# seung-lab/crackle

Hardware: AMD Instinct MI355X
Metric: voxels/s encode+decode, 1024x1024x512 uint32; bit-exact .ckl bytes (higher is better)
Workload: dtype u32

## Files before the change

crackle_amd/csrc/ckl_encode.hip:

```cpp
#include "ckl_common.hpp"
#include "ckl_runs.hpp"
#include "ckl_trail.hpp"
#include "ckl_pins_dev.hpp"

#include <algorithm>
#include <atomic>
#include <chrono>
#include <functional>
#include <memory>
#include <mutex>

namespace ckl {

using namespace dev;

template <typename LABEL>
__global__ void __launch_bounds__(kBlock) k_stats(const LABEL* __restrict__ labels, uint64_t voxels, unsigned long long* __restrict__ out ) {
	__shared__ unsigned long long s_max[kWaves], s_pairs[kWaves];
	unsigned long long mx = 0, pairs = 0;
	const uint64_t stride = static_cast<uint64_t>(gridDim.x) * kBlock;
	for (uint64_t i = static_cast<uint64_t>(blockIdx.x) * kBlock + threadIdx.x; i < voxels; i += stride) {
		const LABEL v = labels[i];
		if (static_cast<unsigned long long>(v) > mx) mx = v;
		if (i > 0) pairs += (labels[i - 1] == v);
// ... 631 lines not shown
	uint32_t b = planeV[wi];
	if (w == 0) b |= 1u;
	const uint32_t* cc = run_cc + rbase[zi];
	const uint32_t add = static_cast<uint32_t>(comp_off[zi]) + id_base;
	uint32_t run = word_base[wi] - 1u + __popc(b & (0xFFFFFFFFu >> (31u - bit)));
	uint4 o;
	o.x = cc[run] + add;
	run += (b >> (bit + 1u)) & 1u; o.y = cc[run] + add;
	run += (b >> (bit + 2u)) & 1u; o.z = cc[run] + add;
	run += (b >> (bit + 3u)) & 1u; o.w = cc[run] + add;
	*reinterpret_cast<uint4*>(out + zi * sxy + px) = o;
}

inline void launch_paint_components(hipStream_t s, const uint32_t* planeV, uint32_t row_words, uint64_t plane_words, int64_t sx, int64_t sy, int64_t sz,
	const uint32_t* word_base, const uint64_t* rbase, const uint32_t* run_cc, const uint64_t* comp_off, uint32_t id_base, uint32_t* out) {
	const uint64_t sxy = static_cast<uint64_t>(sx) * sy;
	const bool four = sx % 4 == 0 && (reinterpret_cast<uintptr_t>(out) & 15u) == 0;
	const uint64_t threads = four ? sxy / 4 : sxy;
	const dim3 grid(static_cast<uint32_t>((threads + kBlock - 1) / kBlock), static_cast<uint32_t>(sz));
	if (four) hipLaunchKernelGGL(k_paint_components4, grid, dim3(kBlock), 0, s, planeV, row_words, plane_words, static_cast<uint32_t>(sx), sxy, word_base, rbase, run_cc, comp_off, id_base, out);
	else hipLaunchKernelGGL(k_paint_components, grid, dim3(kBlock), 0, s, planeV, row_words, plane_words, static_cast<uint32_t>(sx), sxy, word_base, rbase, run_cc, comp_off, id_base, out);
}

__global__ void __launch_bounds__(kBlock) k_bitonic_step(uint64_t* __restrict__ a, uint32_t j, uint32_t k, uint32_t n) {
	const uint32_t i = blockIdx.x * kBlock + threadIdx.x;
	if (i >= n) return;
	const uint32_t l = i ^ j;
	if (l > i) {
		const uint64_t x = a[i], y = a[l];
		const bool up = (i & k) == 0;
		if ((x > y) == up) { a[i] = y; a[l] = x; }
	}
}
__global__ void __launch_bounds__(kBlock) k_bitonic_step2(uint64_t* __restrict__ a, uint32_t j, uint32_t k, uint32_t n) {
	const uint32_t t = blockIdx.x * kBlock + threadIdx.x;
	if (t >= n / 4u) return;
	const uint32_t h = j >> 1;
	const uint32_t lb = static_cast<uint32_t>(__ffs(h)) - 1u;
	const uint32_t i = (t & (h - 1u)) | ((t >> lb) << (lb + 2u));
	uint64_t v0 = a[i], v1 = a[i | h], v2 = a[i | j], v3 = a[i | j | h];
	const bool up = (i & k) == 0;
	auto cx = [&](uint64_t& x, uint64_t& y) { if ((x > y) == up) { const uint64_t z = x; x = y; y = z; } };
	cx(v0, v2); cx(v1, v3);
	cx(v0, v1); cx(v2, v3);
	a[i] = v0; a[i | h] = v1; a[i | j] = v2; a[i | j | h] = v3;
}

__global__ void __launch_bounds__(kBlock) k_bitonic_first(uint64_t* __restrict__ a, uint32_t n) {
	__shared__ uint64_t s[2048];
	const uint32_t base = blockIdx.x * 2048u;
	for (uint32_t t = threadIdx.x; t < 2048u; t += kBlock) s[t] = base + t < n ? a[base + t] : ~0ull;
	__syncthreads();
	for (uint32_t k = 2; k <= 2048u; k <<= 1) {
		for (uint32_t j = k >> 1; j > 0; j >>= 1) {
			for (uint32_t t = threadIdx.x; t < 2048u; t += kBlock) {
				const uint32_t l = t ^ j;
				if (l > t) {
					const uint64_t x = s[t], y = s[l];
					const bool up = ((base + t) & k) == 0;
					if ((x > y) == up) { s[t] = y; s[l] = x; }
				}
			}
			__syncthreads();
		}
	}
	for (uint32_t t = threadIdx.x; t < 2048u; t += kBlock) if (base + t < n) a[base + t] = s[t];
}
__global__ void __launch_bounds__(kBlock) k_bitonic_local(uint64_t* __restrict__ a, uint32_t j_start, uint32_t k, uint32_t n) {
	__shared__ uint64_t s[2048];
	const uint32_t base = blockIdx.x * 2048u;
	for (uint32_t t = threadIdx.x; t < 2048u; t += kBlock) s[t] = base + t < n ? a[base + t] : ~0ull;
	__syncthreads();
	for (uint32_t j = j_start; j > 0; j >>= 1) {
		for (uint32_t t = threadIdx.x; t < 2048u; t += kBlock) {
			const uint32_t l = t ^ j;
			if (l > t) {
				const uint64_t x = s[t], y = s[l];
				const bool up = ((base + t) & k) == 0;
				if ((x > y) == up) { s[t] = y; s[l] = x; }
			}
		}
		__syncthreads();
	}
	for (uint32_t t = threadIdx.x; t < 2048u; t += kBlock) if (base + t < n) a[base + t] = s[t];
}
__global__ void __launch_bounds__(kBlock) k_pad_copy_u64(const uint64_t* __restrict__ src, uint64_t n, uint64_t* __restrict__ dst, uint64_t n_pad) {
	const uint64_t i = static_cast<uint64_t>(blockIdx.x) * kBlock + threadIdx.x;
	if (i < n_pad) dst[i] = i < n ? src[i] : ~0ull;
}
constexpr uint32_t kUniqPer = 8, kUniqItems = kBlock * kUniqPer;
__device__ __forceinline__ uint32_t unique_heads(const uint64_t* __restrict__ sorted, uint32_t n, uint32_t i0, uint64_t (&v)[kUniqPer]) {
	uint32_t flag = 0;
#pragma unroll
	for (uint32_t q = 0; q < kUniqPer; q++) {
		const uint32_t i = i0 + q;
		v[q] = i < n ? sorted[i] : 0;
		const uint64_t prev = q ? v[q - 1] : ((i > 0 && i < n) ? sorted[i - 1] : 0);
		flag |= ((i < n && (i == 0 || v[q] != prev)) ? 1u : 0u) << q;
	}
	return flag;
}
__global__ void __launch_bounds__(kBlock) k_unique_count(const uint64_t* __restrict__ sorted, uint32_t n, uint32_t* __restrict__ blk_count) {
	__shared__ uint32_t s_red[kWaves];
	uint64_t v[kUniqPer];
	const uint32_t flag = unique_heads(sorted, n, blockIdx.x * kUniqItems + threadIdx.x * kUniqPer, v);
	const uint32_t tot = block_sum(static_cast<uint32_t>(__popc(flag)), s_red);
	if (threadIdx.x == 0) blk_count[blockIdx.x] = tot;
}
__global__ void __launch_bounds__(kBlock) k_unique_scan(uint32_t* __restrict__ blk_count, uint32_t nblk, uint32_t* __restrict__ n_uniq) {
	__shared__ uint32_t s_scan[kWaves];
	uint32_t carry = 0;
// ... 50 lines not shown
__global__ void __launch_bounds__(kBlock) k_label_hash_count(const unsigned long long* __restrict__ table, uint32_t slots, uint32_t* __restrict__ blk_count) {
	__shared__ uint32_t s_red[kWaves];
	uint64_t v[kUniqPer];
	const uint32_t flag = hash_occupied(table, slots, blockIdx.x * kUniqItems + threadIdx.x * kUniqPer, v);
	const uint32_t tot = block_sum(static_cast<uint32_t>(__popc(flag)), s_red);
	if (threadIdx.x == 0) blk_count[blockIdx.x] = tot;
}
__global__ void __launch_bounds__(kBlock) k_label_hash_scatter(
	const unsigned long long* __restrict__ table, uint32_t slots, const uint32_t* __restrict__ blk_base, const uint32_t* __restrict__ n_found,
	const uint32_t* __restrict__ has_max, uint64_t* __restrict__ out
) {
	__shared__ uint32_t s_scan[kWaves];
	uint64_t v[kUniqPer];
	const uint32_t flag = hash_occupied(table, slots, blockIdx.x * kUniqItems + threadIdx.x * kUniqPer, v);
	uint32_t c[1] = { static_cast<uint32_t>(__popc(flag)) }, tot[1];
	block_excl_add<1>(c, tot, s_scan);
	uint32_t o = blk_base[blockIdx.x] + c[0];
#pragma unroll
	for (uint32_t q = 0; q < kUniqPer; q++) if ((flag >> q) & 1u) out[o++] = v[q];
	if (blockIdx.x == 0 && threadIdx.x == 0 && *has_max) out[*n_found] = kLabelHashEmpty;
}

__global__ void __launch_bounds__(kBlock) k_flat_section(
	const uint64_t* __restrict__ uniq, const uint32_t* __restrict__ n_uniq, int stored_width,
	const uint32_t* __restrict__ ncomp, uint32_t nslices, int component_width,
	const uint64_t* __restrict__ mapping, uint32_t n, uint8_t* __restrict__ out
) {
	const uint32_t nu = *n_uniq;
	const int key_width = nu <= 0xFFu ? 1 : (nu <= 0xFFFFu ? 2 : 4);
	const uint32_t i = blockIdx.x * kBlock + threadIdx.x;
	if (i == 0) for (int b = 0; b < 8; b++) out[b] = static_cast<uint8_t>((static_cast<uint64_t>(nu) >> (8 * b)) & 0xFF);
	uint8_t* o_uniq = out + 8;
	uint8_t* o_cc = o_uniq + static_cast<uint64_t>(nu) * stored_width;
	uint8_t* o_keys = o_cc + static_cast<uint64_t>(nslices) * component_width;
	if (i < nu) {
		const uint64_t v = uniq[i];
		for (int b = 0; b < stored_width; b++) o_uniq[static_cast<uint64_t>(i) * stored_width + b] = static_cast<uint8_t>((v >> (8 * b)) & 0xFF);
	}
	if (i < nslices) {
		const uint32_t v = ncomp[i];
		for (int b = 0; b < component_width; b++) o_cc[static_cast<uint64_t>(i) * component_width + b] = b < 4 ? static_cast<uint8_t>((v >> (8 * b)) & 0xFF) : 0;
	}
	if (i < n) {
		const uint64_t v = mapping[i];
		uint32_t lo = 0, hi = nu;
		while (lo + 1 < hi) {
			const uint32_t mid = (lo + hi) >> 1;
			if (uniq[mid] <= v) lo = mid; else hi = mid;
		}
		for (int b = 0; b < key_width; b++) o_keys[static_cast<uint64_t>(i) * key_width + b] = static_cast<uint8_t>((lo >> (8 * b)) & 0xFF);
	}
// ... 170 lines not shown
	hipStream_t stream_tab = nullptr;
	hipEvent_t ev_codes = nullptr;
	void* tables_staging = nullptr;
	bool uploads_by_kernel = false;
	hipEvent_t ev_labels_crc = nullptr;
	DevBuf<uint32_t> d_labels_crc;
	DevBuf<uint8_t> d_stream_out;
	uint64_t device_stream_bytes = 0;
	uint64_t last_codes_total = 0;
	DevBuf<uint32_t> d_stack_node, d_stack_code;
	DevBuf<uint32_t> d_chain_node, d_chain_off, d_chain_clen, d_chain_order, d_chain_dst, d_chain_vstart;
	DevBuf<uint32_t> d_n_chains, d_n_raw, d_n_valid, d_payload_len, d_boc_len;
	DevBuf<uint32_t> d_hist;
	DevBuf<uint32_t> d_planes, d_count_vh;
	uint32_t row_words = 0;
	uint64_t plane_words = 0;
	std::vector<uint32_t> count_v, count_h;
	DevBuf<uint64_t> d_rbase;
	DevBuf<uint32_t> d_rcap, d_word_base, d_parent, d_run_start, d_run_cc, d_comp_pix, d_nruns, d_ncomp, d_idbits, d_blk_roots;
	DevBuf<uint16_t> d_run_local;
	DevBuf<uint32_t> d_G, d_crc_acc;
	DevBuf<uint32_t> d_flat_report;
	uint64_t g_table_pixels = 0;
	DevBuf<uint64_t> d_mapping, d_sorted, d_uniq, d_label_hash, d_label_list;
	DevBuf<uint8_t> d_keys;
	DevBuf<uint32_t> d_cc_volume;
	DevBuf<uint32_t> d_pin_kept, d_pin_u32;
	DevBuf<uint8_t> d_pin_tables;
	DevBuf<uint64_t> d_pin_u64;
	DevBuf<uint32_t> d_slice_err2, d_n_uniq, d_uniq_blk;
	DevBuf<uint8_t> d_labels_bin;
	uint32_t flat_max_rcap = 0;
	const void* planes_for = nullptr;
	const void* trail_for = nullptr;
	bool trail_perm = false;
	int trail_order = 0;
	VolumeStats planes_stats;
	int64_t planes_dims[3] = { 0, 0, 0 };
	std::vector<uint64_t> h_rbase;
	std::vector<uint32_t> h_rcap;
	std::vector<uint32_t> count_special, count_corner;
	DevBuf<uint32_t> d_plane_partial, t_blk_special, t_blk_corner;
	DevBuf<unsigned long long> d_plane_partial_max, d_plane_out;
	uint32_t graph_blocks = 0;
	uint32_t tiles_x = 0, tiles_y = 0, mtx2 = 0;
	uint64_t adjm_stride = 0;
	bool graph_permissible = false;
	bool planes_deferred = false;
	bool trail_zeroed = false;
	DevBuf<uint64_t> t_nbase, t_cobase, t_ibase;
	DevBuf<uint32_t> t_ncap, t_cocap, t_icap, t_max_steps;
	size_t last_trail_slices = 0;
	DevBuf<uint32_t> t_counters;
	DevBuf<uint32_t> t_node_vertex, t_vert2node, t_corner_vertex;
	DevBuf<uint8_t> t_node_adj;
	DevBuf<uint32_t> t_dart_end, t_dart_len, t_dart_minv, t_dart_minpos, t_parent, t_start_bits, t_starts;
	DevBuf<uint4> t_dart_codes;
	DevBuf<uint8_t> t_dart_inline;
	DevBuf<unsigned long long> t_compmin;
	DevBuf<uint32_t> t_items, t_item_off, t_chain_item0, t_events, t_chain_ev0, t_ev_lnd, t_ev_item;

	~ckl_encoder() {
		if (ev0) (void)hipEventDestroy(ev0);
		if (ev1) (void)hipEventDestroy(ev1);
		if (evk0) (void)hipEventDestroy(evk0);
		if (evk1) (void)hipEventDestroy(evk1);
		if (evd0) (void)hipEventDestroy(evd0);
		if (evd1) (void)hipEventDestroy(evd1);
		if (ev_in) (void)hipEventDestroy(ev_in);
		if (ev_prezero) (void)hipEventDestroy(ev_prezero);
		if (stream) (void)hipStreamDestroy(stream);
		if (stream2) (void)hipStreamDestroy(stream2);
		if (stream_copy) { (void)hipStreamSynchronize(stream_copy); (void)hipStreamDestroy(stream_copy); }
		if (stream_tab) { (void)hipStreamSynchronize(stream_tab); (void)hipStreamDestroy(stream_tab); }
		if (ev_codes) (void)hipEventDestroy(ev_codes);
		if (tables_staging) host_out_free(tables_staging);
		if (ev_labels_crc) (void)hipEventDestroy(ev_labels_crc);
	}
};

namespace {

template <typename T>
void upload(DevBuf<T>& d, const std::vector<T>& h, hipStream_t s) {
	d.ensure(h.size());
	if (!h.empty()) CKL_HIP(hipMemcpyAsync(d.p, h.data(), h.size() * sizeof(T), hipMemcpyHostToDevice, s));
}
struct UploadPacker {
	struct Item { void* buf; size_t off, count; void (*bind)(void*, uint8_t*, size_t); };
	std::vector<Item> items;
	std::vector<uint8_t> image;
	template <typename T>
	void add(DevBuf<T>& dst, const std::vector<T>& src) {
		const size_t off = (image.size() + 255) & ~static_cast<size_t>(255);
		image.resize(off + std::max<size_t>(src.size(), 1) * sizeof(T));
// ... 527 lines not shown
		const std::vector<uint32_t> rep = download(e.d_flat_report.p, 4 * static_cast<size_t>(ns), s);
		out.ncomp.assign(rep.begin(), rep.begin() + ns);
		acc.assign(rep.begin() + ns, rep.begin() + 2 * static_cast<size_t>(ns));
		idbits.assign(rep.begin() + 2 * static_cast<size_t>(ns), rep.begin() + 3 * static_cast<size_t>(ns));
		errs.assign(rep.begin() + 3 * static_cast<size_t>(ns), rep.end());
		HT_MARK("f:wait");
	}
	else {
		out.ncomp = download(e.d_ncomp.p, ns, s);
		HT_MARK("f:wait");
		acc = download(e.d_crc_acc.p, ns, s);
		idbits = download(e.d_idbits.p, ns, s);
		errs = download(e.d_slice_err2.p, ns, s);
	}
	for (uint32_t zi = 0; zi < ns; zi++) if (errs[zi]) throw Error(CKL_ERR_RUNTIME, "crackle_amd: run table overflow on z=" + std::to_string(zi));
	const uint32_t init_term = gf_mul(0xFFFFFFFFu, gf_xpow(32ull * sxy));
	out.crcs.resize(ns);
	uint32_t fix_bits = 0xFFFFFFFFu, fix = 0;
	for (uint32_t zi = 0; zi < ns; zi++) {
		if (idbits[zi] != fix_bits) { fix_bits = idbits[zi]; fix = gf_xpow(32 - fix_bits); }
		out.crcs[zi] = ~(gf_mul(acc[zi], fix) ^ init_term);
	}

	std::vector<uint64_t> comp_off(ns);
	uint64_t total = 0;
	for (uint32_t zi = 0; zi < ns; zi++) { comp_off[zi] = total; total += out.ncomp[zi]; }
	upload(e.d_comp_off, comp_off, s);
	e.d_mapping.ensure(total + 1);
	RunArrays ra;
	ra.word_base = e.d_word_base.p; ra.rbase = e.d_rbase.p; ra.rcap = e.d_rcap.p;
	ra.parent = e.d_parent.p; ra.run_start = e.d_run_start.p; ra.run_cc = e.d_run_cc.p;
	ra.nruns = e.d_nruns.p; ra.ncomp = e.d_ncomp.p; ra.slice_err = e.d_slice_err2.p;
	ra.comp_pix = e.d_comp_pix.p;
	uint32_t max_ncomp = 1;
	for (uint32_t zi = 0; zi < ns; zi++) max_ncomp = std::max(max_ncomp, out.ncomp[zi]);
	hipLaunchKernelGGL(k_mapping_comps<LABEL>, dim3((max_ncomp + kBlock - 1) / kBlock, ns), dim3(kBlock), 0, s,
		labels, ra, sxy, e.d_comp_off.p, e.d_mapping.p);
	CKL_HIP(hipStreamSynchronize(s));
	out.total = total;
}

struct PinLabelLists {
	DevBuf<uint64_t> d_tab;
	DevBuf<uint32_t> d_count;
	uint32_t slots = 0;
	hipEvent_t ready = nullptr;
	~PinLabelLists() { if (ready) (void)hipEventDestroy(ready); }
};
void pin_label_table_enqueue(ckl_encoder& e, const uint64_t* comp_label, const uint64_t* first_any_dev, uint64_t N, PinLabelLists& t) {
	hipStream_t s = e.stream2;
	if (N > (1ull << 30)) throw Error(CKL_ERR_RUNTIME, "crackle_amd: too many components for pin labels");
	uint32_t slots = 1024;
	while (slots < 2 * N) slots <<= 1;
	t.slots = slots;
	t.d_tab.ensure(4ull * slots + 1);
	t.d_count.ensure(1);
	CKL_HIP(hipMemsetAsync(t.d_tab.p, 0xFF, (2ull * slots) * sizeof(uint64_t), s));
	CKL_HIP(hipMemsetAsync(t.d_tab.p + 4ull * slots, 0xFF, sizeof(uint64_t), s));
	CKL_HIP(hipMemsetAsync(t.d_count.p, 0, sizeof(uint32_t), s));
	unsigned long long* tab = reinterpret_cast<unsigned long long*>(t.d_tab.p);
	hipLaunchKernelGGL(k_pin_label_first, dim3(static_cast<uint32_t>((N + kPinBlock - 1) / kPinBlock)), dim3(kPinBlock), 0, s,
// ... 346 lines not shown
		pin_label_table_collect(e, lists, lc);
		HT_MARK("p:lists");
		table = pins_label_table_host(lc.label_value, lc.label_first);
		HT_MARK("p:table");
	}
	const uint64_t total = download(d_off.p + N, 1, s)[0];
	HT_MARK("p:passes");
	uint64_t id_budget = 1ull << 26;
	if (const char* env = getenv("CKL_PIN_IDS_BUDGET")) id_budget = static_cast<uint64_t>(std::max(0, atoi(env)));
	if (total > id_budget || getenv("CKL_PINS_HOST_BOOKKEEPING")) {
		const PinCandidates pc = pin_candidates_device<LABEL>(e, labels, cc, comp_label, sx, sy, sz, N, &v, choice, first_any);
		HT_MARK("pins_device");
		return pins_cover_host(pc, sx, sy, sz, nc, N, index_width, stored_width, auto_bgcolor, manual_bgcolor);
	}
	d_ze.ensure(N); d_ids.ensure(total + 1);
	hipLaunchKernelGGL(k_pin_minus1, dim3(nb), dim3(kPinBlock), 0, s, d_zep.p, N, d_ze.p);
	hipLaunchKernelGGL(k_pin_ids, dim3(nb), dim3(kPinBlock), 0, s, v, choice, d_ze.p, reinterpret_cast<const uint64_t*>(d_off.p), static_cast<uint32_t>(N), d_ids.p);
	std::vector<uint8_t> bin = pins_section_from_device(e, sx, sy, sz, N, nc, comp_label, first_any, reinterpret_cast<const uint64_t*>(choice), d_zep.p,
		reinterpret_cast<const uint64_t*>(d_off.p), d_ids.p, stored_width, auto_bgcolor, manual_bgcolor, table.get());
	HT_MARK("pins_host");
	return bin;
}

uint64_t flat_section(ckl_encoder& e, uint64_t N, int stored_width, int component_width, uint32_t ns, const ckl_encode_overrides* ov = nullptr) {
	hipStream_t s = e.stream2;
	if (N > 0x7FFFFFFFull) throw Error(CKL_ERR_RUNTIME, "crackle_amd: too many components");
	e.d_n_uniq.ensure(2);
	e.d_uniq.ensure(N + 1);
	const uint64_t* sort_src = e.d_mapping.p;
	uint64_t n_sort = N;
	if (N > 8192 && N <= (1ull << 26) && !getenv("CKL_LABEL_SORT_ALL")) {
		uint32_t slots = 16384;
		while (slots < 2 * N) slots <<= 1;
		e.d_label_hash.ensure(slots);
		CKL_HIP(hipMemsetAsync(e.d_label_hash.p, 0xFF, static_cast<size_t>(slots) * sizeof(uint64_t), s));
		CKL_HIP(hipMemsetAsync(e.d_n_uniq.p, 0, 2 * sizeof(uint32_t), s));
		unsigned long long* table = reinterpret_cast<unsigned long long*>(e.d_label_hash.p);
		hipLaunchKernelGGL(k_label_hash_insert, dim3(static_cast<uint32_t>((N + kBlock - 1) / kBlock)), dim3(kBlock), 0, s, e.d_mapping.p, static_cast<uint32_t>(N), table, slots - 1u, e.d_n_uniq.p + 1);
		const uint32_t hb = (slots + kUniqItems - 1) / kUniqItems;
		e.d_uniq_blk.ensure(hb + 1);
		hipLaunchKernelGGL(k_label_hash_count, dim3(hb), dim3(kBlock), 0, s, table, slots, e.d_uniq_blk.p);
		hipLaunchKernelGGL(k_unique_scan, dim3(1), dim3(kBlock), 0, s, e.d_uniq_blk.p, hb, e.d_n_uniq.p);
		hipLaunchKernelGGL(k_label_hash_scatter, dim3(hb), dim3(kBlock), 0, s, table, slots, e.d_uniq_blk.p, e.d_n_uniq.p, e.d_n_uniq.p + 1, e.d_uniq.p);
		const std::vector<uint32_t> found = download(e.d_n_uniq.p, 2, s);
		n_sort = static_cast<uint64_t>(found[0]) + (found[1] ? 1u : 0u);
		if (n_sort == 0 || n_sort > N) throw Error(CKL_ERR_RUNTIME, "crackle_amd: label table pass failed");
		e.d_label_list.ensure(n_sort);
		CKL_HIP(hipMemcpyAsync(e.d_label_list.p, e.d_uniq.p, n_sort * sizeof(uint64_t), hipMemcpyDeviceToDevice, s));
		sort_src = e.d_label_list.p;
	}
	const bool merge_unsorted = ov && ov->merge_unique && sort_src == e.d_label_list.p;
	uint32_t n_pad = 2048;
	while (n_pad < n_sort) n_pad <<= 1;
	if (!merge_unsorted) {
	e.d_sorted.ensure(n_pad);
	const uint32_t blocks = (n_pad + kBlock - 1) / kBlock;
	hipLaunchKernelGGL(k_pad_copy_u64, dim3(blocks), dim3(kBlock), 0, s, sort_src, n_sort, e.d_sorted.p, static_cast<uint64_t>(n_pad));
	hipLaunchKernelGGL(k_bitonic_first, dim3(n_pad / 2048), dim3(kBlock), 0, s, e.d_sorted.p, n_pad);
	for (uint32_t k = 4096; k <= n_pad; k <<= 1) {
		uint32_t j = k >> 1;
		for (; j >= 4096 && !getenv("CKL_BITONIC_SINGLE_STEPS"); j >>= 2) hipLaunchKernelGGL(k_bitonic_step2, dim3((n_pad / 4 + kBlock - 1) / kBlock), dim3(kBlock), 0, s, e.d_sorted.p, j, k, n_pad);
		for (; j >= 2048; j >>= 1) hipLaunchKernelGGL(k_bitonic_step, dim3(blocks), dim3(kBlock), 0, s, e.d_sorted.p, j, k, n_pad);
		hipLaunchKernelGGL(k_bitonic_local, dim3(n_pad / 2048), dim3(kBlock), 0, s, e.d_sorted.p, j, k, n_pad);
	}
	{
		const uint32_t ub = static_cast<uint32_t>((n_sort + kUniqItems - 1) / kUniqItems);
		e.d_uniq_blk.ensure(ub + 1);
		hipLaunchKernelGGL(k_unique_count, dim3(ub), dim3(kBlock), 0, s, e.d_sorted.p, static_cast<uint32_t>(n_sort), e.d_uniq_blk.p);
		hipLaunchKernelGGL(k_unique_scan, dim3(1), dim3(kBlock), 0, s, e.d_uniq_blk.p, ub, e.d_n_uniq.p);
		hipLaunchKernelGGL(k_unique_scatter, dim3(ub), dim3(kBlock), 0, s, e.d_sorted.p, static_cast<uint32_t>(n_sort), e.d_uniq_blk.p, e.d_uniq.p);
	}
	}
	uint64_t uniq_bound = N;
	if (ov && ov->merge_unique) {
		HT_MARK("l:enqueue");
		const uint32_t n_local = merge_unsorted ? static_cast<uint32_t>(n_sort) : download(e.d_n_uniq.p, 1, s)[0];
		std::vector<uint64_t> local = download(merge_unsorted ? e.d_label_list.p : e.d_uniq.p, n_local, s);
		HT_MARK("l:local");
		const uint64_t* merged = nullptr;
		uint64_t n_merged = 0;
		if (ov->merge_unique(ov->merge_ctx, local.data(), n_local, &merged, &n_merged) != 0 || (!merged && n_merged))
			throw Error(CKL_ERR_RUNTIME, "crackle_amd: the merge_unique callback failed");
		HT_MARK("l:merge");
		if (n_merged < n_local || n_merged > 0xFFFFFFFFull) throw Error(CKL_ERR_ARG, "crackle_amd: merge_unique returned a list that cannot contain the slab's labels");
		e.d_uniq.ensure(n_merged + 1);
		if (n_merged) CKL_HIP(hipMemcpyAsync(e.d_uniq.p, merged, n_merged * sizeof(uint64_t), hipMemcpyHostToDevice, s));
		const uint32_t nm = static_cast<uint32_t>(n_merged);
		CKL_HIP(hipMemcpyAsync(e.d_n_uniq.p, &nm, sizeof(uint32_t), hipMemcpyHostToDevice, s));
		CKL_HIP(hipStreamSynchronize(s));
		e.d_labels_bin.ensure(8 + n_merged * static_cast<uint64_t>(stored_width) + static_cast<uint64_t>(ns) * component_width + N * 4 + 16);
		uniq_bound = std::max<uint64_t>(uniq_bound, n_merged);
	}
	e.d_labels_bin.ensure(8 + N * static_cast<uint64_t>(stored_width) + static_cast<uint64_t>(ns) * component_width + N * 4 + 16);
	const uint64_t work = std::max<uint64_t>(std::max<uint64_t>(uniq_bound, ns), 1);
	hipLaunchKernelGGL(k_flat_section, dim3(static_cast<uint32_t>((work + kBlock - 1) / kBlock)), dim3(kBlock), 0, s,
		e.d_uniq.p, e.d_n_uniq.p, stored_width, e.d_ncomp.p, ns, component_width, e.d_mapping.p, static_cast<uint32_t>(N), e.d_labels_bin.p);
	HT_MARK("l:enqueue");
	const uint32_t nu = download(e.d_n_uniq.p, 1, s)[0];
	HT_MARK("l:wait");
	return 8 + static_cast<uint64_t>(nu) * stored_width + static_cast<uint64_t>(ns) * component_width + N * static_cast<uint64_t>(byte_width(nu));
}

template <typename LABEL>
void encode_typed(
	ckl_encoder& e, const LABEL* labels, int64_t sx, int64_t sy, int64_t sz,
	bool allow_pins, bool fortran_order, uint64_t markov_model_order,
	bool optimize_pins, bool auto_bgcolor, int64_t manual_bgcolor,
	const ckl_encode_overrides* ov, uint8_t** out, uint64_t* out_len
) {
	const uint64_t voxels = static_cast<uint64_t>(sx) * sy * sz;
	hipStream_t s = e.stream;
	CKL_HIP(hipEventRecord(e.ev0, s));

	HostTimer ht;
	g_ht = &ht;
	VolumeStats st;
	e.trail_zeroed = false;
	const bool planes_cached = ov && voxels > 0 && e.planes_for == static_cast<const void*>(labels)
		&& e.planes_dims[0] == sx && e.planes_dims[1] == sy && e.planes_dims[2] == sz;
	e.planes_for = nullptr;
	const bool labels_first = getenv("CKL_NO_OVERLAP") || static_cast<uint64_t>(sx) * sy > (1536ull * 1536ull)
// ... 89 lines not shown
	uint64_t label_bytes = 0;
	const uint64_t off_index = Header::kBytes;
	const uint64_t off_labels = off_index + 4ull * (sz + 1);
	uint64_t est_code_bytes = 0;
	{
		const uint64_t interior = static_cast<uint64_t>(sx > 0 ? sx - 1 : 0) * sy + static_cast<uint64_t>(sx) * (sy > 0 ? sy - 1 : 0);
		const int xw = byte_width(static_cast<uint64_t>(sx) + 1), yw = byte_width(static_cast<uint64_t>(sy) + 1);
		for (int64_t z = 0; z < sz; z++) {
			const uint64_t differ = static_cast<uint64_t>(e.count_v[z]) + e.count_h[z];
			const uint64_t E = permissible ? interior - differ : differ;
			const uint64_t codes = E + 4ull * (static_cast<uint64_t>(e.count_special[z]) + e.count_corner[z]) + 16;
			est_code_bytes += (head.markov_model_order ? (3 * codes + 7) / 8 : (codes + 3) / 4) + 8;
			est_code_bytes += 4 + yw + 64ull * (yw + 2 * xw);
		}
	}
	if (getenv("CKL_SMALL_ESTIMATE")) est_code_bytes = 0;
	const uint64_t model_bytes_est = head.markov_model_order ? (1ull << (2 * head.markov_model_order)) : 0;
	struct HostOut { void* p = nullptr; ~HostOut() { if (p) host_out_free(p); } } early;
	uint64_t early_cap = 0;
	uint32_t labels_crc = 0;
	const int component_width = byte_width(static_cast<uint64_t>(sx) * sy);
	hipStream_t s2 = e.stream2;
	bool labels_stay = false;
	auto label_side = [&]() {
		if (labels_at_walk) {
			CKL_HIP(hipStreamWaitEvent(s2, e.evd0, 0));
			flat_enqueue(e, sx, sy, sz);
		}
		flat_collect<LABEL>(e, labels, sx, sy, sz, fr);
		HT_MARK("flat");
		const uint64_t N = fr.total;
		if (head.label_format == PINS_VARIABLE_WIDTH) {
			if (N > 0xFFFFFFFFull) throw Error(CKL_ERR_RUNTIME, "crackle_amd: too many components");
			e.d_cc_volume.ensure(voxels);
			launch_paint_components(s2, e.d_planes.p, e.row_words, e.plane_words, sx, sy, sz, e.d_word_base.p, e.d_rbase.p, e.d_run_cc.p, e.d_comp_off.p, 0u, e.d_cc_volume.p);
			pins_binary = pins_section_plain<LABEL>(e, labels, e.d_cc_volume.p, e.d_mapping.p, sx, sy, sz, N, fr.ncomp, head.pin_index_width(), stored_width, auto_bgcolor, manual_bgcolor);
			label_bytes = pins_binary.size();
		}
		else {
			label_bytes = flat_section(e, N, stored_width, component_width, static_cast<uint32_t>(sz), ov);
			HT_MARK("label_table");
			labels_stay = e.async_host_copy && e.keep_device_stream && !e.defer_codes && label_bytes > 0;
			early_cap = off_labels + label_bytes + model_bytes_est + est_code_bytes + 4ull * (sz + 1) + 64;
			early.p = host_out_alloc(early_cap);
			HT_MARK("l:buffer");
			uint8_t* eo = static_cast<uint8_t*>(early.p);
// ... 35 lines not shown
	}
	try {
		e.last_codes_total = cr.total;
		if (head.label_format == PINS_VARIABLE_WIDTH) {
			if (label_bytes) memcpy(o + off_labels, pins_binary.data(), label_bytes);
			labels_crc = crc32c(o + off_labels, label_bytes);
		}
		std::vector<uint8_t> hb;
		head.write(hb);
		memcpy(o, hb.data(), hb.size());
		auto put4 = [&](uint64_t at, uint32_t v) { for (int b = 0; b < 4; b++) o[at + b] = static_cast<uint8_t>((v >> (8 * b)) & 0xFF); };
		for (int64_t z = 0; z < sz; z++) put4(off_index + 4ull * z, cr.code_len[z]);
		put4(off_index + 4ull * sz, crc32c(o + off_index, 4ull * sz));
		if (!stored_model.empty()) memcpy(o + off_model, stored_model.data(), stored_model.size());
		for (int64_t z = 0; z < sz; z++) put4(off_tail + 4 + 4ull * z, fr.crcs[z]);
		put4(off_tail, labels_crc);
		e.device_stream_bytes = 0;
		if (e.keep_device_stream) {
			e.d_stream_out.ensure(total + 16);
			uint8_t* ds = e.d_stream_out.p;
			const void* up = head.label_format == FLAT ? o : nullptr;
			upload_small(ds, o, off_labels, s, up);
			if (label_bytes) {
				if (head.label_format == FLAT) copy_bytes_device(e.d_labels_bin.p, ds + off_labels, label_bytes, s);
				else CKL_HIP(hipMemcpyAsync(ds + off_labels, o + off_labels, label_bytes, hipMemcpyHostToDevice, s));
			}
			if (!stored_model.empty()) upload_small(ds + off_model, o + off_model, stored_model.size(), s, up);
			if (cr.total) copy_bytes_device(e.d_codes_out.p, ds + off_codes, cr.total, s);
			upload_small(ds + off_tail, o + off_tail, 4ull * (sz + 1), s, up);
			if (labels_stay) {
				CKL_HIP(hipStreamWaitEvent(s, e.ev_labels_crc, 0));
				CKL_HIP(hipMemcpyAsync(ds + off_tail, e.d_labels_crc.p, 4, hipMemcpyDeviceToDevice, s));
			}
			e.device_stream_bytes = total;
		}
		if (cr.total && !e.defer_codes) {
			if (e.async_host_copy && e.keep_device_stream) {
				if (!e.stream_copy) CKL_HIP(hipStreamCreateWithFlags(&e.stream_copy, hipStreamNonBlocking));
				if (!e.ev_codes) CKL_HIP(hipEventCreateWithFlags(&e.ev_codes, hipEventDisableTiming));
				CKL_HIP(hipEventRecord(e.ev_codes, s));
				CKL_HIP(hipStreamWaitEvent(e.stream_copy, e.ev_codes, 0));
				CKL_HIP(hipMemcpyAsync(o + off_codes, e.d_codes_out.p, cr.total, hipMemcpyDeviceToHost, e.stream_copy));
				if (labels_stay) {
					CKL_HIP(hipMemcpyAsync(o + off_labels, e.d_labels_bin.p, label_bytes, hipMemcpyDeviceToHost, e.stream_copy));
					CKL_HIP(hipMemcpyAsync(o + off_tail, e.d_labels_crc.p, 4, hipMemcpyDeviceToHost, e.stream_copy));
				}
				e.host_copy_pending = true;
			}
			else CKL_HIP(hipMemcpyAsync(o + off_codes, e.d_codes_out.p, cr.total, hipMemcpyDeviceToHost, s));
		}
		ht.mark("assembly");
		CKL_HIP(hipEventRecord(e.ev1, s));
		CKL_HIP(hipStreamSynchronize(s));
		ht.mark("codes_d2h");
		CKL_HIP(hipGetLastError());
		CKL_HIP(hipEventElapsedTime(&e.pipeline_ms, e.ev0, e.ev1));
		CKL_HIP(hipEventElapsedTime(&e.trail_ms, e.evk0, e.evk1));
		CKL_HIP(hipEventElapsedTime(&e.dominant_ms, e.evd0, e.evd1));
	}
	catch (...) {
		if (e.host_copy_pending) { (void)hipStreamSynchronize(e.stream_copy); e.host_copy_pending = false; }
		host_out_free(o);
		throw;
	}
	*out = o;
	*out_len = total;
}

void reencode_markov(const uint8_t* buf, uint64_t n, int markov_order, int device, uint8_t** out, uint64_t* out_len) {
	if (n < Header::kBytesV0) throw Error(CKL_ERR_FORMAT, "crackle: Input too small to be a valid stream. Bytes: " + std::to_string(n));
	Header head = Header::parse(buf, n);
	if (markov_order < 0 || markov_order > 13) throw Error(CKL_ERR_ARG, "crackle_amd: markov_model_order must be in [0, 13] on device");
	auto copy_out = [&](const uint8_t* p, uint64_t len) {
		uint8_t* o = static_cast<uint8_t*>(host_out_alloc(len));
		memcpy(o, p, len);
		*out = o; *out_len = len;
	};
	if (head.markov_model_order == markov_order) { copy_out(buf, n); return; }
	const bool v0 = head.format_version == 0;
	const uint64_t sz = head.sz;
	const uint64_t tail_bytes = v0 ? 0 : 4 * (sz + 1);
	const uint64_t off_index = head.header_bytes();
	const uint64_t off_labels = off_index + head.grid_index_bytes();
	if (!head.layout_fits(n)) throw Error(CKL_ERR_RUNTIME, "crackle: get_crack_code_offsets: Unable to read past end of buffer.");
	const uint64_t old_codes = off_labels + head.num_label_bytes + head.markov_model_bytes();
	uint64_t old_tail = old_codes;
	for (uint64_t z = 0; z < sz; z++) old_tail += rd_le(buf + off_index + 4 * z, 4);
// ... 572 lines not shown
```

Before: 156.3 billion.

## Replace global bitonic sort with block sort plus 8-way merge-path passes

Replaces the padded power-of-two bitonic sort (many global step kernel launches) with a shared-memory 4096-key block sort followed by 8-way merge passes that place each element by binary-searching its rank in the sibling runs. In the hashed path the unique count comes from the host, so the post-sort unique count/scatter and a device-to-device copy are skipped. A host stream sync after the mapping kernel is removed, with RAII draining of the label stream added. This cuts the number of sort launches and passes, in exchange for per-element binary searches with scattered global reads and extra buffers.

```diff
diff --git a/crackle_amd/csrc/ckl_encode.hip b/crackle_amd/csrc/ckl_encode.hip
--- a/crackle_amd/csrc/ckl_encode.hip
+++ b/crackle_amd/csrc/ckl_encode.hip
@@ -677,71 +677,83 @@
 	else hipLaunchKernelGGL(k_paint_components, grid, dim3(kBlock), 0, s, planeV, row_words, plane_words, static_cast<uint32_t>(sx), sxy, word_base, rbase, run_cc, comp_off, id_base, out);
 }
 
-__global__ void __launch_bounds__(kBlock) k_bitonic_step(uint64_t* __restrict__ a, uint32_t j, uint32_t k, uint32_t n) {
-	const uint32_t i = blockIdx.x * kBlock + threadIdx.x;
-	if (i >= n) return;
-	const uint32_t l = i ^ j;
-	if (l > i) {
-		const uint64_t x = a[i], y = a[l];
-		const bool up = (i & k) == 0;
-		if ((x > y) == up) { a[i] = y; a[l] = x; }
-	}
-}
-__global__ void __launch_bounds__(kBlock) k_bitonic_step2(uint64_t* __restrict__ a, uint32_t j, uint32_t k, uint32_t n) {
-	const uint32_t t = blockIdx.x * kBlock + threadIdx.x;
-	if (t >= n / 4u) return;
-	const uint32_t h = j >> 1;
-	const uint32_t lb = static_cast<uint32_t>(__ffs(h)) - 1u;
-	const uint32_t i = (t & (h - 1u)) | ((t >> lb) << (lb + 2u));
-	uint64_t v0 = a[i], v1 = a[i | h], v2 = a[i | j], v3 = a[i | j | h];
-	const bool up = (i & k) == 0;
-	auto cx = [&](uint64_t& x, uint64_t& y) { if ((x > y) == up) { const uint64_t z = x; x = y; y = z; } };
-	cx(v0, v2); cx(v1, v3);
-	cx(v0, v1); cx(v2, v3);
-	a[i] = v0; a[i | h] = v1; a[i | j] = v2; a[i | j | h] = v3;
-}
-
-__global__ void __launch_bounds__(kBlock) k_bitonic_first(uint64_t* __restrict__ a, uint32_t n) {
-	__shared__ uint64_t s[2048];
-	const uint32_t base = blockIdx.x * 2048u;
-	for (uint32_t t = threadIdx.x; t < 2048u; t += kBlock) s[t] = base + t < n ? a[base + t] : ~0ull;
+constexpr uint32_t kSortKeys = 4096, kSortThreads = 1024, kMergeFan = 8;
+__global__ void __launch_bounds__(kSortThreads) k_sort_blocks(const uint64_t* src, uint32_t n, uint64_t* dst) {
+	__shared__ uint64_t s[kSortKeys];
+	const uint32_t base = blockIdx.x * kSortKeys, t = threadIdx.x;
+	for (uint32_t i = t; i < kSortKeys; i += kSortThreads) s[i] = base + i < n ? src[base + i] : ~0ull;
 	__syncthreads();
-	for (uint32_t k = 2; k <= 2048u; k <<= 1) {
-		for (uint32_t j = k >> 1; j > 0; j >>= 1) {
-			for (uint32_t t = threadIdx.x; t < 2048u; t += kBlock) {
-				const uint32_t l = t ^ j;
-				if (l > t) {
-					const uint64_t x = s[t], y = s[l];
-					const bool up = ((base + t) & k) == 0;
-					if ((x > y) == up) { s[t] = y; s[l] = x; }
-				}
+	auto cx = [](uint64_t& x, uint64_t& y, bool up) { if ((x > y) == up) { const uint64_t z = x; x = y; y = z; } };
+	for (uint32_t k = 2; k <= kSortKeys; k <<= 1) {
+		uint32_t j = k >> 1;
+		for (; j >= 2; j >>= 2) {
+			const uint32_t h = j >> 1;
+			const uint32_t lb = static_cast<uint32_t>(__ffs(h)) - 1u;
+			const uint32_t i = (t & (h - 1u)) | ((t >> lb) << (lb + 2u));
+			uint64_t v0 = s[i], v1 = s[i | h], v2 = s[i | j], v3 = s[i | j | h];
+			const bool up = (i & k) == 0;
+			cx(v0, v2, up); cx(v1, v3, up);
+			cx(v0, v1, up); cx(v2, v3, up);
+			s[i] = v0; s[i | h] = v1; s[i | j] = v2; s[i | j | h] = v3;
+			__syncthreads();
+		}
+		if (j == 1) {
+			const uint32_t i = 4u * t;
+			uint64_t v0 = s[i], v1 = s[i + 1], v2 = s[i + 2], v3 = s[i + 3];
+			cx(v0, v1, (i & k) == 0); cx(v2, v3, ((i + 2u) & k) == 0);
+			s[i] = v0; s[i + 1] = v1; s[i + 2] = v2; s[i + 3] = v3;
+			__syncthreads();
+		}
+	}
+	for (uint32_t i = t; i < kSortKeys; i += kSortThreads) if (base + i < n) dst[base + i] = s[i];
+}
+__global__ void __launch_bounds__(kBlock) k_merge_runs(const uint64_t* __restrict__ src, uint32_t n, uint32_t run_len, uint64_t* __restrict__ dst) {
+	__shared__ uint32_t s_lo[kMergeFan], s_hi[kMergeFan];
+	const uint32_t b0 = blockIdx.x * kBlock;
+	const uint32_t run = b0 / run_len, g0 = run / kMergeFan * kMergeFan, own = run - g0;
+	const uint64_t group = static_cast<uint64_t>(g0) * run_len;
+	if (threadIdx.x < 2u * kMergeFan) {
+		const uint32_t q = threadIdx.x >> 1;
+		const bool upper = threadIdx.x & 1u;
+		const uint64_t start = group + static_cast<uint64_t>(q) * run_len;
+		uint32_t lo = 0;
+		if (q != own && start < n) {
+			const uint64_t* a = src + start;
+			const uint64_t x = upper ? src[min(b0 + kBlock, n) - 1u] : src[b0];
+			uint32_t hi = static_cast<uint32_t>(min(static_cast<uint64_t>(run_len), n - start));
+			while (lo < hi) {
+				const uint32_t mid = (lo + hi) >> 1;
+				const uint64_t v = a[mid];
+				if (v < x || (upper && v == x)) lo = mid + 1u; else hi = mid;
 			}
-			__syncthreads();
-		}
-	}
-	for (uint32_t t = threadIdx.x; t < 2048u; t += kBlock) if (base + t < n) a[base + t] = s[t];
-}
-__global__ void __launch_bounds__(kBlock) k_bitonic_local(uint64_t* __restrict__ a, uint32_t j_start, uint32_t k, uint32_t n) {
-	__shared__ uint64_t s[2048];
-	const uint32_t base = blockIdx.x * 2048u;
-	for (uint32_t t = threadIdx.x; t < 2048u; t += kBlock) s[t] = base + t < n ? a[base + t] : ~0ull;
+		}
+		(upper ? s_hi : s_lo)[q] = lo;
+	}
 	__syncthreads();
-	for (uint32_t j = j_start; j > 0; j >>= 1) {
-		for (uint32_t t = threadIdx.x; t < 2048u; t += kBlock) {
-			const uint32_t l = t ^ j;
-			if (l > t) {
-				const uint64_t x = s[t], y = s[l];
-				const bool up = ((base + t) & k) == 0;
-				if ((x > y) == up) { s[t] = y; s[l] = x; }
+	const uint32_t g = b0 + threadIdx.x;
+	if (g >= n) return;
+	const uint64_t x = src[g];
+	uint32_t lo[kMergeFan], len[kMergeFan], live = 0;
+#pragma unroll
+	for (uint32_t q = 0; q < kMergeFan; q++) { lo[q] = s_lo[q]; len[q] = s_hi[q] - lo[q]; live |= len[q]; }
+	while (live) {
+		live = 0;
+#pragma unroll
+		for (uint32_t q = 0; q < kMergeFan; q++) {
+			if (len[q]) {
+				const uint32_t half = len[q] >> 1;
+				const uint64_t v = src[group + static_cast<uint64_t>(q) * run_len + lo[q] + half];
+				const bool right = v < x || (q < own && v == x);
+				lo[q] = right ? lo[q] + half + 1u : lo[q];
+				len[q] = right ? len[q] - half - 1u : half;
 			}
-		}
-		__syncthreads();
-	}
-	for (uint32_t t = threadIdx.x; t < 2048u; t += kBlock) if (base + t < n) a[base + t] = s[t];
-}
-__global__ void __launch_bounds__(kBlock) k_pad_copy_u64(const uint64_t* __restrict__ src, uint64_t n, uint64_t* __restrict__ dst, uint64_t n_pad) {
-	const uint64_t i = static_cast<uint64_t>(blockIdx.x) * kBlock + threadIdx.x;
-	if (i < n_pad) dst[i] = i < n ? src[i] : ~0ull;
+			live |= len[q];
+		}
+	}
+	uint32_t rank = g - run * run_len;
+#pragma unroll
+	for (uint32_t q = 0; q < kMergeFan; q++) rank += lo[q];
+	dst[group + rank] = x;
 }
 constexpr uint32_t kUniqPer = 8, kUniqItems = kBlock * kUniqPer;
 __device__ __forceinline__ uint32_t unique_heads(const uint64_t* __restrict__ sorted, uint32_t n, uint32_t i0, uint64_t (&v)[kUniqPer]) {
@@ -838,11 +850,11 @@
 }
 
 __global__ void __launch_bounds__(kBlock) k_flat_section(
-	const uint64_t* __restrict__ uniq, const uint32_t* __restrict__ n_uniq, int stored_width,
+	const uint64_t* __restrict__ uniq, const uint32_t* __restrict__ n_uniq, uint32_t n_uniq_host, int stored_width,
 	const uint32_t* __restrict__ ncomp, uint32_t nslices, int component_width,
 	const uint64_t* __restrict__ mapping, uint32_t n, uint8_t* __restrict__ out
 ) {
-	const uint32_t nu = *n_uniq;
+	const uint32_t nu = n_uniq ? *n_uniq : n_uniq_host;
 	const int key_width = nu <= 0xFFu ? 1 : (nu <= 0xFFFFu ? 2 : 4);
 	const uint32_t i = blockIdx.x * kBlock + threadIdx.x;
 	if (i == 0) for (int b = 0; b < 8; b++) out[b] = static_cast<uint8_t>((static_cast<uint64_t>(nu) >> (8 * b)) & 0xFF);
@@ -1059,7 +1071,7 @@
 	DevBuf<uint32_t> d_G, d_crc_acc;
 	DevBuf<uint32_t> d_flat_report;
 	uint64_t g_table_pixels = 0;
-	DevBuf<uint64_t> d_mapping, d_sorted, d_uniq, d_label_hash, d_label_list;
+	DevBuf<uint64_t> d_mapping, d_sorted, d_sort_alt, d_uniq, d_label_hash, d_label_list;
 	DevBuf<uint8_t> d_keys;
 	DevBuf<uint32_t> d_cc_volume;
 	DevBuf<uint32_t> d_pin_kept, d_pin_u32;
@@ -1074,7 +1086,7 @@
 	int trail_order = 0;
 	VolumeStats planes_stats;
 	int64_t planes_dims[3] = { 0, 0, 0 };
-	std::vector<uint64_t> h_rbase;
+	std::vector<uint64_t> h_rbase, h_comp_off;
 	std::vector<uint32_t> h_rcap;
 	std::vector<uint32_t> count_special, count_corner;
 	DevBuf<uint32_t> d_plane_partial, t_blk_special, t_blk_corner;
@@ -1107,7 +1119,7 @@
 		if (ev_in) (void)hipEventDestroy(ev_in);
 		if (ev_prezero) (void)hipEventDestroy(ev_prezero);
 		if (stream) (void)hipStreamDestroy(stream);
-		if (stream2) (void)hipStreamDestroy(stream2);
+		if (stream2) { (void)hipStreamSynchronize(stream2); (void)hipStreamDestroy(stream2); }
 		if (stream_copy) { (void)hipStreamSynchronize(stream_copy); (void)hipStreamDestroy(stream_copy); }
 		if (stream_tab) { (void)hipStreamSynchronize(stream_tab); (void)hipStreamDestroy(stream_tab); }
 		if (ev_codes) (void)hipEventDestroy(ev_codes);
@@ -1681,7 +1693,8 @@
 		out.crcs[zi] = ~(gf_mul(acc[zi], fix) ^ init_term);
 	}
 
-	std::vector<uint64_t> comp_off(ns);
+	std::vector<uint64_t>& comp_off = e.h_comp_off;
+	comp_off.resize(ns);
 	uint64_t total = 0;
 	for (uint32_t zi = 0; zi < ns; zi++) { comp_off[zi] = total; total += out.ncomp[zi]; }
 	upload(e.d_comp_off, comp_off, s);
@@ -1695,7 +1708,6 @@
 	for (uint32_t zi = 0; zi < ns; zi++) max_ncomp = std::max(max_ncomp, out.ncomp[zi]);
 	hipLaunchKernelGGL(k_mapping_comps<LABEL>, dim3((max_ncomp + kBlock - 1) / kBlock, ns), dim3(kBlock), 0, s,
 		labels, ra, sxy, e.d_comp_off.p, e.d_mapping.p);
-	CKL_HIP(hipStreamSynchronize(s));
 	out.total = total;
 }
 
@@ -2088,17 +2100,32 @@
 	return bin;
 }
 
+static const uint64_t* sort_keys_device(const uint64_t* src, uint32_t n, uint64_t* a, uint64_t* b, hipStream_t s) {
+	hipLaunchKernelGGL(k_sort_blocks, dim3((n + kSortKeys - 1) / kSortKeys), dim3(kSortThreads), 0, s, src, n, a);
+	for (uint64_t run_len = kSortKeys; run_len < n; run_len *= kMergeFan) {
+		hipLaunchKernelGGL(k_merge_runs, dim3((n + kBlock - 1) / kBlock), dim3(kBlock), 0, s, a, n, static_cast<uint32_t>(run_len), b);
+		std::swap(a, b);
+	}
+	return a;
+}
+
 uint64_t flat_section(ckl_encoder& e, uint64_t N, int stored_width, int component_width, uint32_t ns, const ckl_encode_overrides* ov = nullptr) {
 	hipStream_t s = e.stream2;
 	if (N > 0x7FFFFFFFull) throw Error(CKL_ERR_RUNTIME, "crackle_amd: too many components");
 	e.d_n_uniq.ensure(2);
-	e.d_uniq.ensure(N + 1);
-	const uint64_t* sort_src = e.d_mapping.p;
+	const bool merging = ov && ov->merge_unique;
+	const uint64_t* uniq = nullptr;
+	const uint32_t* d_nu = e.d_n_uniq.p;
+	uint32_t nu_host = 0;
+	uint64_t uniq_bound = N;
+	bool hashed = false;
 	uint64_t n_sort = N;
 	if (N > 8192 && N <= (1ull << 26) && !getenv("CKL_LABEL_SORT_ALL")) {
+		hashed = true;
 		uint32_t slots = 16384;
 		while (slots < 2 * N) slots <<= 1;
 		e.d_label_hash.ensure(slots);
+		e.d_sorted.ensure(N + 1);
 		CKL_HIP(hipMemsetAsync(e.d_label_hash.p, 0xFF, static_cast<size_t>(slots) * sizeof(uint64_t), s));
 		CKL_HIP(hipMemsetAsync(e.d_n_uniq.p, 0, 2 * sizeof(uint32_t), s));
 		unsigned long long* table = reinterpret_cast<unsigned long long*>(e.d_label_hash.p);
@@ -2107,41 +2134,38 @@
 		e.d_uniq_blk.ensure(hb + 1);
 		hipLaunchKernelGGL(k_label_hash_count, dim3(hb), dim3(kBlock), 0, s, table, slots, e.d_uniq_blk.p);
 		hipLaunchKernelGGL(k_unique_scan, dim3(1), dim3(kBlock), 0, s, e.d_uniq_blk.p, hb, e.d_n_uniq.p);
-		hipLaunchKernelGGL(k_label_hash_scatter, dim3(hb), dim3(kBlock), 0, s, table, slots, e.d_uniq_blk.p, e.d_n_uniq.p, e.d_n_uniq.p + 1, e.d_uniq.p);
+		hipLaunchKernelGGL(k_label_hash_scatter, dim3(hb), dim3(kBlock), 0, s, table, slots, e.d_uniq_blk.p, e.d_n_uniq.p, e.d_n_uniq.p + 1, e.d_sorted.p);
 		const std::vector<uint32_t> found = download(e.d_n_uniq.p, 2, s);
 		n_sort = static_cast<uint64_t>(found[0]) + (found[1] ? 1u : 0u);
 		if (n_sort == 0 || n_sort > N) throw Error(CKL_ERR_RUNTIME, "crackle_amd: label table pass failed");
-		e.d_label_list.ensure(n_sort);
-		CKL_HIP(hipMemcpyAsync(e.d_label_list.p, e.d_uniq.p, n_sort * sizeof(uint64_t), hipMemcpyDeviceToDevice, s));
-		sort_src = e.d_label_list.p;
-	}
-	const bool merge_unsorted = ov && ov->merge_unique && sort_src == e.d_label_list.p;
-	uint32_t n_pad = 2048;
-	while (n_pad < n_sort) n_pad <<= 1;
-	if (!merge_unsorted) {
-	e.d_sorted.ensure(n_pad);
-	const uint32_t blocks = (n_pad + kBlock - 1) / kBlock;
-	hipLaunchKernelGGL(k_pad_copy_u64, dim3(blocks), dim3(kBlock), 0, s, sort_src, n_sort, e.d_sorted.p, static_cast<uint64_t>(n_pad));
-	hipLaunchKernelGGL(k_bitonic_first, dim3(n_pad / 2048), dim3(kBlock), 0, s, e.d_sorted.p, n_pad);
-	for (uint32_t k = 4096; k <= n_pad; k <<= 1) {
-		uint32_t j = k >> 1;
-		for (; j >= 4096 && !getenv("CKL_BITONIC_SINGLE_STEPS"); j >>= 2) hipLaunchKernelGGL(k_bitonic_step2, dim3((n_pad / 4 + kBlock - 1) / kBlock), dim3(kBlock), 0, s, e.d_sorted.p, j, k, n_pad);
-		for (; j >= 2048; j >>= 1) hipLaunchKernelGGL(k_bitonic_step, dim3(blocks), dim3(kBlock), 0, s, e.d_sorted.p, j, k, n_pad);
-		hipLaunchKernelGGL(k_bitonic_local, dim3(n_pad / 2048), dim3(kBlock), 0, s, e.d_sorted.p, j, k, n_pad);
-	}
-	{
+	}
+	if (hashed && !merging) {
+		e.d_uniq.ensure(N + 1);
+		uniq = sort_keys_device(e.d_sorted.p, static_cast<uint32_t>(n_sort), e.d_sorted.p, e.d_uniq.p, s);
+		d_nu = nullptr;
+		nu_host = static_cast<uint32_t>(n_sort);
+	}
+	else if (!hashed) {
+		e.d_sorted.ensure(N); e.d_sort_alt.ensure(N); e.d_uniq.ensure(N + 1);
 		const uint32_t ub = static_cast<uint32_t>((n_sort + kUniqItems - 1) / kUniqItems);
 		e.d_uniq_blk.ensure(ub + 1);
-		hipLaunchKernelGGL(k_unique_count, dim3(ub), dim3(kBlock), 0, s, e.d_sorted.p, static_cast<uint32_t>(n_sort), e.d_uniq_blk.p);
-		hipLaunchKernelGGL(k_unique_scan, dim3(1), dim3(kBlock), 0, s, e.d_uniq_blk.p, ub, e.d_n_uniq.p);
-		hipLaunchKernelGGL(k_unique_scatter, dim3(ub), dim3(kBlock), 0, s, e.d_sorted.p, static_cast<uint32_t>(n_sort), e.d_uniq_blk.p, e.d_uniq.p);
-	}
-	}
-	uint64_t uniq_bound = N;
-	if (ov && ov->merge_unique) {
+		if (n_sort) {
+			const uint64_t* sorted = sort_keys_device(e.d_mapping.p, static_cast<uint32_t>(n_sort), e.d_sorted.p, e.d_sort_alt.p, s);
+			hipLaunchKernelGGL(k_unique_count, dim3(ub), dim3(kBlock), 0, s, sorted, static_cast<uint32_t>(n_sort), e.d_uniq_blk.p);
+			hipLaunchKernelGGL(k_unique_scan, dim3(1), dim3(kBlock), 0, s, e.d_uniq_blk.p, ub, e.d_n_uniq.p);
+			hipLaunchKernelGGL(k_unique_scatter, dim3(ub), dim3(kBlock), 0, s, sorted, static_cast<uint32_t>(n_sort), e.d_uniq_blk.p, e.d_uniq.p);
+		}
+		else CKL_HIP(hipMemsetAsync(e.d_n_uniq.p, 0, sizeof(uint32_t), s));
+		uniq = e.d_uniq.p;
+	}
+	if (merging) {
 		HT_MARK("l:enqueue");
-		const uint32_t n_local = merge_unsorted ? static_cast<uint32_t>(n_sort) : download(e.d_n_uniq.p, 1, s)[0];
-		std::vector<uint64_t> local = download(merge_unsorted ? e.d_label_list.p : e.d_uniq.p, n_local, s);
+		const uint32_t n_local = hashed ? static_cast<uint32_t>(n_sort) : download(e.d_n_uniq.p, 1, s)[0];
+		if (hashed) {
+			e.d_label_list.ensure(n_sort);
+			CKL_HIP(hipMemcpyAsync(e.d_label_list.p, e.d_sorted.p, n_sort * sizeof(uint64_t), hipMemcpyDeviceToDevice, s));
+		}
+		std::vector<uint64_t> local = download(hashed ? e.d_label_list.p : e.d_uniq.p, n_local, s);
 		HT_MARK("l:local");
 		const uint64_t* merged = nullptr;
 		uint64_t n_merged = 0;
@@ -2151,18 +2175,18 @@
 		if (n_merged < n_local || n_merged > 0xFFFFFFFFull) throw Error(CKL_ERR_ARG, "crackle_amd: merge_unique returned a list that cannot contain the slab's labels");
 		e.d_uniq.ensure(n_merged + 1);
 		if (n_merged) CKL_HIP(hipMemcpyAsync(e.d_uniq.p, merged, n_merged * sizeof(uint64_t), hipMemcpyHostToDevice, s));
-		const uint32_t nm = static_cast<uint32_t>(n_merged);
-		CKL_HIP(hipMemcpyAsync(e.d_n_uniq.p, &nm, sizeof(uint32_t), hipMemcpyHostToDevice, s));
 		CKL_HIP(hipStreamSynchronize(s));
-		e.d_labels_bin.ensure(8 + n_merged * static_cast<uint64_t>(stored_width) + static_cast<uint64_t>(ns) * component_width + N * 4 + 16);
+		uniq = e.d_uniq.p;
+		d_nu = nullptr;
+		nu_host = static_cast<uint32_t>(n_merged);
 		uniq_bound = std::max<uint64_t>(uniq_bound, n_merged);
 	}
-	e.d_labels_bin.ensure(8 + N * static_cast<uint64_t>(stored_width) + static_cast<uint64_t>(ns) * component_width + N * 4 + 16);
+	e.d_labels_bin.ensure(8 + uniq_bound * static_cast<uint64_t>(stored_width) + static_cast<uint64_t>(ns) * component_width + N * 4 + 16);
 	const uint64_t work = std::max<uint64_t>(std::max<uint64_t>(uniq_bound, ns), 1);
 	hipLaunchKernelGGL(k_flat_section, dim3(static_cast<uint32_t>((work + kBlock - 1) / kBlock)), dim3(kBlock), 0, s,
-		e.d_uniq.p, e.d_n_uniq.p, stored_width, e.d_ncomp.p, ns, component_width, e.d_mapping.p, static_cast<uint32_t>(N), e.d_labels_bin.p);
+		uniq, d_nu, nu_host, stored_width, e.d_ncomp.p, ns, component_width, e.d_mapping.p, static_cast<uint32_t>(N), e.d_labels_bin.p);
 	HT_MARK("l:enqueue");
-	const uint32_t nu = download(e.d_n_uniq.p, 1, s)[0];
+	const uint32_t nu = d_nu ? download(d_nu, 1, s)[0] : nu_host;
 	HT_MARK("l:wait");
 	return 8 + static_cast<uint64_t>(nu) * stored_width + static_cast<uint64_t>(ns) * component_width + N * static_cast<uint64_t>(byte_width(nu));
 }
@@ -2298,6 +2322,7 @@
 	const int component_width = byte_width(static_cast<uint64_t>(sx) * sy);
 	hipStream_t s2 = e.stream2;
 	bool labels_stay = false;
+	struct StreamDrain { hipStream_t s; bool armed = true; ~StreamDrain() { if (armed) (void)hipStreamSynchronize(s); } } drain_labels{ s2 };
 	auto label_side = [&]() {
 		if (labels_at_walk) {
 			CKL_HIP(hipStreamWaitEvent(s2, e.evd0, 0));
@@ -2379,16 +2404,14 @@
 			const void* up = head.label_format == FLAT ? o : nullptr;
 			upload_small(ds, o, off_labels, s, up);
 			if (label_bytes) {
+				if (labels_stay) CKL_HIP(hipStreamWaitEvent(s, e.ev_labels_crc, 0));
 				if (head.label_format == FLAT) copy_bytes_device(e.d_labels_bin.p, ds + off_labels, label_bytes, s);
 				else CKL_HIP(hipMemcpyAsync(ds + off_labels, o + off_labels, label_bytes, hipMemcpyHostToDevice, s));
 			}
 			if (!stored_model.empty()) upload_small(ds + off_model, o + off_model, stored_model.size(), s, up);
 			if (cr.total) copy_bytes_device(e.d_codes_out.p, ds + off_codes, cr.total, s);
 			upload_small(ds + off_tail, o + off_tail, 4ull * (sz + 1), s, up);
-			if (labels_stay) {
-				CKL_HIP(hipStreamWaitEvent(s, e.ev_labels_crc, 0));
-				CKL_HIP(hipMemcpyAsync(ds + off_tail, e.d_labels_crc.p, 4, hipMemcpyDeviceToDevice, s));
-			}
+			if (labels_stay) CKL_HIP(hipMemcpyAsync(ds + off_tail, e.d_labels_crc.p, 4, hipMemcpyDeviceToDevice, s));
 			e.device_stream_bytes = total;
 		}
 		if (cr.total && !e.defer_codes) {
@@ -2420,6 +2443,7 @@
 		host_out_free(o);
 		throw;
 	}
+	drain_labels.armed = false;
 	*out = o;
 	*out_len = total;
 }
```

Result: no change. 156.6 billion (median of 3 runs) (+0.2%).
